# aluo7/ViT-SOM

Measured on AMD Instinct MI355X. Metric: images/sec/node ViT-SOM 40x40 CIFAR-10 bs512 (training step: fwd+bwd+all-reduce+AdamW), higher is better.
Workload: dtype f32 (Linear GEMMs on bf16 MFMA: forward from an exact 3xbf16 operand split, six products; weight / input gradients from a 2xbf16 split, three products, rel. error 4e-6)

## Files before the change

vit_som_amd/csrc/attention.hip:

```cpp
#include "common.h"
#include "attention_layout.h"

#include <atomic>

#include <stdlib.h>

#pragma clang fp contract(off)

namespace vsom {

int gemm_grad_products();

static std::atomic<int> g_attn_fused{1};

#ifdef VSOM_ATTN_STAMPS
__device__ unsigned long long* g_attn_stamps = nullptr;
#define ATTN_STAMP(i)                                                                              \
    do {                                                                                           \
        if (threadIdx.x == 0 && g_attn_stamps) g_attn_stamps[blockIdx.x * 16 + (i)] = __builtin_amdgcn_s_memrealtime(); \
    } while (0)
#define ATTN_STAMP_HWID()                                                                          \
    do {                                                                                           \
        if (threadIdx.x == 0 && g_attn_stamps) {                                                   \
            unsigned hw, xcc;                                                                      \
            asm volatile("s_getreg_b32 %0, hwreg(HW_REG_HW_ID)" : "=s"(hw));                       \
            asm volatile("s_getreg_b32 %0, hwreg(HW_REG_XCC_ID)" : "=s"(xcc));                     \
            g_attn_stamps[blockIdx.x * 16 + 4] = hw;                                                \
            g_attn_stamps[blockIdx.x * 16 + 5] = xcc;                                               \
        }                                                                                          \
    } while (0)
#else
#define ATTN_STAMP(i)
#define ATTN_STAMP_HWID()
#endif


template <int HDP>
struct ACfg {
    static constexpr bool VEC = (HDP % 16 == 0);
    static constexpr int S = HDP + 4;
    static constexpr int NMM = HDP / 4;
    static constexpr int NDT = (HDP + 15) / 16;
    static __device__ __forceinline__ int off(int row, int col) { return row * S + col; }
};

__device__ __forceinline__ f32x4 mfma16(float a, float b, f32x4 c) {
    return __builtin_amdgcn_mfma_f32_16x16x4f32(a, b, c, 0, 0, 0);
}

typedef __attribute__((ext_vector_type(8))) __bf16 abf16x8;
typedef __attribute__((ext_vector_type(2))) __bf16 abf16x2;
struct SplitFrag { abf16x8 hi[2], lo[2]; };
__device__ __forceinline__ void split8(const float (&v)[8], abf16x8& hi, abf16x8& lo) {
    unsigned h[4], l[4];
#pragma unroll
    for (int e = 0; e < 4; ++e) {
        const abf16x2 a = {(__bf16)v[2 * e], (__bf16)v[2 * e + 1]};
        const unsigned u = __builtin_bit_cast(unsigned, a);
        const float r0 = v[2 * e] - __uint_as_float(u << 16), r1 = v[2 * e + 1] - __uint_as_float(u & 0xffff0000u);
        const abf16x2 b = {(__bf16)r0, (__bf16)r1};
        h[e] = u; l[e] = __builtin_bit_cast(unsigned, b);
    }
    typedef unsigned u32x4v __attribute__((ext_vector_type(4)));
    hi = __builtin_bit_cast(abf16x8, (u32x4v){h[0], h[1], h[2], h[3]});
    lo = __builtin_bit_cast(abf16x8, (u32x4v){l[0], l[1], l[2], l[3]});
}
__device__ __forceinline__ void split_frag(const float (&f)[16], SplitFrag& o) {
#pragma unroll
    for (int m = 0; m < 2; ++m) {
        float v[8];
#pragma unroll
        for (int j = 0; j < 8; ++j) v[j] = f[8 * m + j];
        split8(v, o.hi[m], o.lo[m]);
    }
}
__device__ __forceinline__ void accum_x3_pair(f32x4 (&o)[4], const float* Zlds, int rowa, int rowb, int r, int qp, f32x4 pa, f32x4 pb) {
    const float pv[8] = {pa[0], pa[1], pa[2], pa[3], pb[0], pb[1], pb[2], pb[3]};
    abf16x8 bh, bl;
    split8(pv, bh, bl);
#pragma unroll
    for (int dt = 0; dt < 4; ++dt) {
        float zv[8];
#pragma unroll
        for (int j = 0; j < 4; ++j) {
            zv[j] = Zlds[ACfg<64>::off(rowa + 4 * qp + j, 16 * dt + r)];
            zv[4 + j] = Zlds[ACfg<64>::off(rowb + 4 * qp + j, 16 * dt + r)];
        }
        abf16x8 ah, al;
        split8(zv, ah, al);
        o[dt] = __builtin_amdgcn_mfma_f32_16x16x32_bf16(al, bh, o[dt], 0, 0, 0);
        o[dt] = __builtin_amdgcn_mfma_f32_16x16x32_bf16(ah, bl, o[dt], 0, 0, 0);
        o[dt] = __builtin_amdgcn_mfma_f32_16x16x32_bf16(ah, bh, o[dt], 0, 0, 0);
    }
}
__device__ __forceinline__ f32x4 score_x3(const SplitFrag& a, const SplitFrag& b) {
    f32x4 acc = {0.f, 0.f, 0.f, 0.f};
#pragma unroll
    for (int m = 0; m < 2; ++m) {
        acc = __builtin_amdgcn_mfma_f32_16x16x32_bf16(a.lo[m], b.hi[m], acc, 0, 0, 0);
        acc = __builtin_amdgcn_mfma_f32_16x16x32_bf16(a.hi[m], b.lo[m], acc, 0, 0, 0);
        acc = __builtin_amdgcn_mfma_f32_16x16x32_bf16(a.hi[m], b.hi[m], acc, 0, 0, 0);
    }
    return acc;
}
struct SplitFrag3 { abf16x8 hi[2], lo[2], rest[2]; };
__device__ __forceinline__ void split_frag3(const float (&f)[16], SplitFrag3& o) {
#pragma unroll
    for (int m = 0; m < 2; ++m) {
        float v[8], w[8];
#pragma unroll
        for (int j = 0; j < 8; ++j) v[j] = f[8 * m + j];
        split8(v, o.hi[m], o.lo[m]);
        const abf16x8 h = o.hi[m], l = o.lo[m];
        abf16x8 t;
#pragma unroll
        for (int j = 0; j < 8; ++j) { w[j] = (v[j] - (float)h[j]) - (float)l[j]; t[j] = (__bf16)w[j]; }
        o.rest[m] = t;
    }
}
__device__ __forceinline__ f32x4 score_x6(const SplitFrag3& a, const SplitFrag3& b) {
    f32x4 acc = {0.f, 0.f, 0.f, 0.f};
#pragma unroll
    for (int m = 0; m < 2; ++m) {
        acc = __builtin_amdgcn_mfma_f32_16x16x32_bf16(a.rest[m], b.hi[m], acc, 0, 0, 0);
        acc = __builtin_amdgcn_mfma_f32_16x16x32_bf16(a.hi[m], b.rest[m], acc, 0, 0, 0);
        acc = __builtin_amdgcn_mfma_f32_16x16x32_bf16(a.lo[m], b.lo[m], acc, 0, 0, 0);
        acc = __builtin_amdgcn_mfma_f32_16x16x32_bf16(a.lo[m], b.hi[m], acc, 0, 0, 0);
        acc = __builtin_amdgcn_mfma_f32_16x16x32_bf16(a.hi[m], b.lo[m], acc, 0, 0, 0);
        acc = __builtin_amdgcn_mfma_f32_16x16x32_bf16(a.hi[m], b.hi[m], acc, 0, 0, 0);
    }
    return acc;
}
typedef SplitFrag3 ScoreFrag;
__device__ __forceinline__ void split_score(const float (&f)[16], ScoreFrag& o) { split_frag3(f, o); }
__device__ __forceinline__ f32x4 score_qk(const ScoreFrag& a, const ScoreFrag& b) { return score_x6(a, b); }
typedef unsigned u32x2 __attribute__((ext_vector_type(2)));
__device__ __forceinline__ void swap16(float v, float& a, float& b) {
    const u32x2 t = __builtin_amdgcn_permlane16_swap(__float_as_uint(v), __float_as_uint(v), false, false);
    a = __uint_as_float(t[0]); b = __uint_as_float(t[1]);
}
__device__ __forceinline__ void swap32(float v, float& a, float& b) {
    const u32x2 t = __builtin_amdgcn_permlane32_swap(__float_as_uint(v), __float_as_uint(v), false, false);
    a = __uint_as_float(t[0]); b = __uint_as_float(t[1]);
}
__device__ __forceinline__ float group_sum(float v) {
    float a, b;
    swap16(v, a, b); v = a + b;
    swap32(v, a, b); return a + b;
}
__device__ __forceinline__ float group_max(float v) {
    float a, b;
    swap16(v, a, b); v = fmaxf(a, b);
    swap32(v, a, b); return fmaxf(a, b);
}
template <int CTRL>
__device__ __forceinline__ float dpp_row(float v) {
    return __int_as_float(__builtin_amdgcn_update_dpp(0, __float_as_int(v), CTRL, 0xf, 0xf, false));
}
__device__ __forceinline__ float tile_sum(float v) {
    v += dpp_row<0x128>(v); v += dpp_row<0x124>(v); v += dpp_row<0x122>(v); v += dpp_row<0x121>(v);
    return v;
}
__device__ __forceinline__ float tile_max(float v) {
    v = fmaxf(v, dpp_row<0x128>(v)); v = fmaxf(v, dpp_row<0x124>(v));
    v = fmaxf(v, dpp_row<0x122>(v)); v = fmaxf(v, dpp_row<0x121>(v));
    return v;
}
__device__ __forceinline__ float wave_sum64(float v) { return group_sum(tile_sum(v)); }
template <bool EXTRA>
__device__ __forceinline__ int tok(int t, int r) { return (EXTRA ? 1 : 0) + 16 * t + r; }

template <int HDP>
__device__ __forceinline__ void stage_rows(float* lds, const float* __restrict__ src, long rs, int N, int nrows,
                                           int hd) {
    constexpr int S = ACfg<HDP>::S;
// ... 91 lines not shown
#pragma unroll
            for (int s = 0; s < 4; ++s) f[4 * g + s] = v[s];
        }
    } else {
#pragma unroll
        for (int mm = 0; mm < ACfg<HDP>::NMM; ++mm) {
            const int d = 4 * mm + qp;
            f[mm] = (ok && d < hd) ? rowptr[d] : 0.f;
        }
    }
}

template <int HDP>
__device__ __forceinline__ void load_frag_lds(float (&f)[ACfg<HDP>::NMM], const float* Y, int row, int qp) {
    if constexpr (ACfg<HDP>::VEC) {
#pragma unroll
        for (int g = 0; g < HDP / 16; ++g) {
            const f32x4 v = *reinterpret_cast<const f32x4*>(Y + ACfg<HDP>::off(row, 16 * g + 4 * qp));
#pragma unroll
            for (int s = 0; s < 4; ++s) f[4 * g + s] = v[s];
        }
    } else {
        load_frag<HDP>(f, Y + row * ACfg<HDP>::S, qp, true, HDP);
    }
}

template <int HDP>
__device__ __forceinline__ f32x4 score_tile(const float* Ylds, int row0, int r, int qp,
                                            const float (&bf)[ACfg<HDP>::NMM]) {
    float af[ACfg<HDP>::NMM];
    load_frag_lds<HDP>(af, Ylds, row0 + r, qp);
    f32x4 acc = {0.f, 0.f, 0.f, 0.f};
#pragma unroll
    for (int mm = 0; mm < ACfg<HDP>::NMM; ++mm) acc = mfma16(af[mm], bf[mm], acc);
    return acc;
}
template <int HDP>
__device__ __forceinline__ void score_tile2(const float* Y0, int row0, const float (&b0)[ACfg<HDP>::NMM], const float* Y1,
                                            int row1, const float (&b1)[ACfg<HDP>::NMM], int r, int qp, f32x4& acc0,
                                            f32x4& acc1) {
    float a0[ACfg<HDP>::NMM], a1[ACfg<HDP>::NMM];
    load_frag_lds<HDP>(a0, Y0, row0 + r, qp);
    load_frag_lds<HDP>(a1, Y1, row1 + r, qp);
    acc0 = f32x4{0.f, 0.f, 0.f, 0.f};
    acc1 = f32x4{0.f, 0.f, 0.f, 0.f};
#pragma unroll
    for (int mm = 0; mm < ACfg<HDP>::NMM; ++mm) {
        acc0 = mfma16(a0[mm], b0[mm], acc0);
        acc1 = mfma16(a1[mm], b1[mm], acc1);
    }
}

template <int HDP>
__device__ __forceinline__ void accum_tile(f32x4 (&o)[ACfg<HDP>::NDT], const float* Zlds, int row0, int r, int qp,
                                           f32x4 p) {
#pragma unroll
    for (int s = 0; s < 4; ++s) {
#pragma unroll
        for (int dt = 0; dt < ACfg<HDP>::NDT; ++dt) {
            float a = 0.f;
            if (ACfg<HDP>::VEC || 16 * dt + r < HDP) a = Zlds[ACfg<HDP>::off(row0 + 4 * qp + s, 16 * dt + r)];
            o[dt] = mfma16(a, p[s], o[dt]);
        }
    }
}
template <int HDP>
__device__ __forceinline__ void accum_tile2(f32x4 (&o0)[ACfg<HDP>::NDT], const float* Z0, f32x4 p0,
                                            f32x4 (&o1)[ACfg<HDP>::NDT], const float* Z1, f32x4 p1, int row0, int r,
                                            int qp) {
#pragma unroll
    for (int s = 0; s < 4; ++s) {
#pragma unroll
        for (int dt = 0; dt < ACfg<HDP>::NDT; ++dt) {
            float a0 = 0.f, a1 = 0.f;
            if (ACfg<HDP>::VEC || 16 * dt + r < HDP) {
                a0 = Z0[ACfg<HDP>::off(row0 + 4 * qp + s, 16 * dt + r)];
                a1 = Z1[ACfg<HDP>::off(row0 + 4 * qp + s, 16 * dt + r)];
            }
            o0[dt] = mfma16(a0, p0[s], o0[dt]);
            o1[dt] = mfma16(a1, p1[s], o1[dt]);
        }
    }
}

template <int HDP>
__device__ __forceinline__ void store_rows(const f32x4 (&o)[ACfg<HDP>::NDT], float* dst, int qp, bool ok, int hd) {
    if (!ok) return;
#pragma unroll
    for (int dt = 0; dt < ACfg<HDP>::NDT; ++dt) {
        const int d0 = 16 * dt + 4 * qp;
        if constexpr (ACfg<HDP>::VEC) {
            *reinterpret_cast<f32x4*>(dst + d0) = o[dt];
        } else {
#pragma unroll
            for (int e = 0; e < 4; ++e)
                if (d0 + e < hd) dst[d0 + e] = o[dt][e];
        }
    }
}

template <int HDP>
__device__ __forceinline__ float frag_dot_row(const float (&f)[ACfg<HDP>::NMM], const float* rowptr, int qp) {
    float y[ACfg<HDP>::NMM];
    load_frag<HDP>(y, rowptr, qp, true, HDP);
    float s = 0.f;
#pragma unroll
    for (int mm = 0; mm < ACfg<HDP>::NMM; ++mm) s = fmaf(f[mm], y[mm], s);
    return group_sum(s);
}
template <int HDP>
__device__ __forceinline__ void axpy_row(f32x4 (&o)[ACfg<HDP>::NDT], float w, const float* rowptr, int qp) {
#pragma unroll
    for (int dt = 0; dt < ACfg<HDP>::NDT; ++dt) {
        const int d0 = 16 * dt + 4 * qp;
        f32x4 v = {0.f, 0.f, 0.f, 0.f};
        if constexpr (ACfg<HDP>::VEC) {
            v = *reinterpret_cast<const f32x4*>(rowptr + d0);
        } else {
#pragma unroll
            for (int e = 0; e < 4; ++e)
                if (d0 + e < HDP) v[e] = rowptr[d0 + e];
        }
        o[dt] += w * v;
    }
}
template <int HDP>
__device__ __forceinline__ float tile_rows_dot(const float* x, const float* Y, int row0, int r, int qp) {
    float xf[ACfg<HDP>::NMM], y[ACfg<HDP>::NMM];
    load_frag<HDP>(xf, x, qp, true, HDP);
    load_frag_lds<HDP>(y, Y, row0 + r, qp);
    float s = 0.f;
#pragma unroll
    for (int mm = 0; mm < ACfg<HDP>::NMM; ++mm) s = fmaf(xf[mm], y[mm], s);
    return group_sum(s);
}
template <int HDP>
__device__ __forceinline__ float tile_wsum(float w, const float* Z, int row0, int lane) {
    float acc = 0.f;
#pragma unroll 4
    for (int j = 0; j < 16; ++j) {
        const float wj = __int_as_float(__builtin_amdgcn_readlane(__float_as_int(w), j));
        if (HDP >= 64 || lane < HDP) acc = fmaf(wj, Z[ACfg<HDP>::off(row0 + j, lane)], acc);
    }
    return acc;
}
template <int HDP>
__device__ __forceinline__ float vec_dot(const float* x, const float* y, int lane) {
    return wave_sum64((HDP >= 64 || lane < HDP) ? x[lane] * y[lane] : 0.f);
}
template <int HDP>
__device__ __forceinline__ float tok0_dq_partial(const float* q0f, const float* do0f, const float* Ks, const float* Vs, int row0, float l0, float D0,
                                                 float scale, int lane, int r, int qp) {
    const float sc = tile_rows_dot<HDP>(q0f, Ks, row0, r, qp);
    const float dp = tile_rows_dot<HDP>(do0f, Vs, row0, r, qp);
    const float w = __expf(sc * scale - l0) * (dp - D0) * scale;
    return tile_wsum<HDP>(w, Ks, row0, lane);
}
template <int HDP>
__device__ __forceinline__ void tok0_dq_combine(const float* q0, const float* do0, const float* k0, const float* v0,
                                                const float* PA, int pa_stride, int nwaves, float l0, float D0,
                                                float scale, float* dst, int hd, int lane) {
    const float s00 = vec_dot<HDP>(q0, k0, lane);
    const float dp00 = vec_dot<HDP>(do0, v0, lane);
    const float w00 = __expf(s00 * scale - l0) * (dp00 - D0) * scale;
    if (HDP >= 64 || lane < HDP) {
        float g = w00 * k0[lane];
        for (int w = 0; w < nwaves; ++w) g += PA[w * pa_stride + lane];
        if (lane < hd) dst[lane] = g;
    }
}
template <int HDP>
__device__ __forceinline__ void tok0_dkv_partial(const float* k0f, const float* v0f, const float* Qs, const float* Ds, const float* Ls, const float* Es,
                                                 int row0, float scale, int lane, int r, int qp, float& gk, float& gv) {
    const float sc = tile_rows_dot<HDP>(k0f, Qs, row0, r, qp);
    const float dp = tile_rows_dot<HDP>(v0f, Ds, row0, r, qp);
    const float p = __expf(sc * scale - Ls[row0 + r]);
    const float ds = p * (dp - Es[row0 + r]) * scale;
    gv += tile_wsum<HDP>(p, Ds, row0, lane);
    gk += tile_wsum<HDP>(ds, Qs, row0, lane);
}
template <int HDP>
__device__ __forceinline__ void tok0_dkv_combine(const float* q0, const float* do0, const float* k0, const float* v0,
                                                 const float* PA, int pa_stride, int nwaves, float l0, float D0,
                                                 float scale, float* dk_dst, float* dv_dst, int hd, int lane) {
    const float s00 = vec_dot<HDP>(q0, k0, lane);
    const float dp00 = vec_dot<HDP>(do0, v0, lane);
    const float p00 = __expf(s00 * scale - l0);
    const float ds00 = p00 * (dp00 - D0) * scale;
    if (HDP >= 64 || lane < HDP) {
        float gk = ds00 * q0[lane], gv = p00 * do0[lane];
        for (int w = 0; w < nwaves; ++w) {
            gk += PA[w * pa_stride + lane];
            gv += PA[w * pa_stride + HDP + lane];
        }
        if (lane < hd) {
            dk_dst[lane] = gk;
            dv_dst[lane] = gv;
        }
    }
}

template <int HDP>
__device__ __forceinline__ float rows_dot(const float (&a)[ACfg<HDP>::NMM], const float (&b)[ACfg<HDP>::NMM]) {
    float D = 0.f;
#pragma unroll
    for (int mm = 0; mm < ACfg<HDP>::NMM; ++mm) D = fmaf(a[mm], b[mm], D);
    return group_sum(D);
}
template <int HDP>
__device__ __forceinline__ void dq_key0(f32x4 (&dq)[ACfg<HDP>::NDT], const float (&qf)[ACfg<HDP>::NMM],
                                        const float (&dof)[ACfg<HDP>::NMM], const float* Ks, const float* Vs, float lq, float D,
                                        float scale, int qp) {
    const float s0 = frag_dot_row<HDP>(qf, Ks, qp) * scale;
    const float dp0 = frag_dot_row<HDP>(dof, Vs, qp);
    const float p0 = __expf(s0 - lq);
    axpy_row<HDP>(dq, p0 * (dp0 - D) * scale, Ks, qp);
}
template <int HDP, bool EXTRA>
__device__ __forceinline__ void dq_scores(f32x4& p, f32x4& ds, const float (&qf)[ACfg<HDP>::NMM],
                                          const float (&dof)[ACfg<HDP>::NMM], const float* Ks, const float* Vs, int t, int N,
                                          bool qok, float lq, float D, float scale, int r, int qp) {
    f32x4 s, dp;
    score_tile2<HDP>(Ks, tok<EXTRA>(t, 0), qf, Vs, tok<EXTRA>(t, 0), dof, r, qp, s, dp);
#pragma unroll
    for (int e = 0; e < 4; ++e) {
        const int key = tok<EXTRA>(t, 4 * qp + e);
        p[e] = (EXTRA || (key < N && qok)) ? __expf(s[e] * scale - lq) : 0.f;
        ds[e] = p[e] * (dp[e] - D) * scale;
    }
}
template <int HDP, bool EXTRA>
__device__ __forceinline__ void dq_tile(f32x4 (&dq)[ACfg<HDP>::NDT], const float (&qf)[ACfg<HDP>::NMM],
                                        const float (&dof)[ACfg<HDP>::NMM], const float* Ks, const float* Vs, int ntile, int N,
                                        bool qok, float lq, float D, float scale, int r, int qp) {
#pragma unroll
    for (int dt = 0; dt < ACfg<HDP>::NDT; ++dt) dq[dt] = f32x4{0.f, 0.f, 0.f, 0.f};
    if (EXTRA) dq_key0<HDP>(dq, qf, dof, Ks, Vs, lq, D, scale, qp);
    for (int t = 0; t < ntile; ++t) {
        f32x4 p, ds;
        dq_scores<HDP, EXTRA>(p, ds, qf, dof, Ks, Vs, t, N, qok, lq, D, scale, r, qp);
        accum_tile<HDP>(dq, Ks, tok<EXTRA>(t, 0), r, qp, ds);
    }
}
template <int HDP, bool EXTRA>
__device__ __forceinline__ void dkv_tile(f32x4 (&dk)[ACfg<HDP>::NDT], f32x4 (&dv)[ACfg<HDP>::NDT],
                                         const float (&kf)[ACfg<HDP>::NMM], const float (&vf)[ACfg<HDP>::NMM], const float* Qs,
                                         const float* Ds, const float* Ls, const float* Es, int ntile, int N, bool kok,
                                         float scale, int r, int qp) {
#pragma unroll
    for (int dt = 0; dt < ACfg<HDP>::NDT; ++dt) { dk[dt] = f32x4{0.f, 0.f, 0.f, 0.f}; dv[dt] = f32x4{0.f, 0.f, 0.f, 0.f}; }
    if (EXTRA) {
        const float s0 = frag_dot_row<HDP>(kf, Qs, qp) * scale;
        const float dp0 = frag_dot_row<HDP>(vf, Ds, qp);
        const float p0 = __expf(s0 - Ls[0]);
        axpy_row<HDP>(dv, p0, Ds, qp);
        axpy_row<HDP>(dk, p0 * (dp0 - Es[0]) * scale, Qs, qp);
    }
    for (int t = 0; t < ntile; ++t) {
        f32x4 s, dp;
        score_tile2<HDP>(Qs, tok<EXTRA>(t, 0), kf, Ds, tok<EXTRA>(t, 0), vf, r, qp, s, dp);
        f32x4 p, ds;
#pragma unroll
// ... 319 lines not shown
    {
        const int q0 = tok<EXTRA>(wave, r);
        load_frag<HDP>(qf, base + (long)q0 * E3, qp, q0 < N, hd);
        load_frag<HDP>(dof, dout + obase + (long)q0 * E, qp, q0 < N, hd);
        load_frag<HDP>(of, out + obase + (long)q0 * E, qp, q0 < N, hd);
    }
    float o0 = 0.f;
    if (EXTRA && lane < hd) o0 = out[obase + lane];
    float l_r = 0.f;
    if ((int)threadIdx.x < N) l_r = lse[srow0 + threadIdx.x];
    stage_rows_quad<HDP>(Ks, base + E, E3, Vs, base + 2 * E, E3, Qs, base, E3, Ds, dout + obase, E, N, nrows);
    for (int i = threadIdx.x; i < nrp; i += blockDim.x) {
        Ls[i] = (i == (int)threadIdx.x) ? l_r : ((i < N) ? lse[srow0 + i] : 0.f);
        Es[i] = 0.f;
    }
    __syncthreads();
    ATTN_STAMP(1);
#ifdef VSOM_ATTN_REPEAT
    for (int rep_ = 0; rep_ < VSOM_ATTN_REPEAT; ++rep_) {
    __syncthreads();
#endif

    float D0 = 0.f, l0 = 0.f, gq0 = 0.f;
    if (EXTRA) {
        D0 = wave_sum64((HDP >= 64 || lane < HDP) ? Ds[lane] * o0 : 0.f);
        l0 = Ls[0];
        if (wave == 0 && lane == 0) { delta[srow0] = D0; Es[0] = D0; }
    }
    for (int qt = wave; qt < ntile; qt += nwaves) {
        const int query = tok<EXTRA>(qt, r);
        const bool qok = query < N;
        if (qt != wave) {
            load_frag<HDP>(qf, base + (long)query * E3, qp, qok, hd);
            load_frag<HDP>(dof, dout + obase + (long)query * E, qp, qok, hd);
            load_frag<HDP>(of, out + obase + (long)query * E, qp, qok, hd);
        }
        const float D = rows_dot<HDP>(dof, of);
        if (qp == 0 && qok) { delta[srow0 + query] = D; Es[query] = D; }
        const float lq = qok ? Ls[query] : 0.f;
        f32x4 dq[NDT];
        dq_tile<HDP, EXTRA>(dq, qf, dof, Ks, Vs, ntile, N, qok, lq, D, scale, r, qp);
        store_rows<HDP>(dq, dqkv + ((long)b * N + query) * E3 + h * hd, qp, qok, hd);
        if (EXTRA) gq0 += tok0_dq_partial<HDP>(Qs, Ds, Ks, Vs, tok<EXTRA>(qt, 0), l0, D0, scale, lane, r, qp);
    }
    if (EXTRA && (HDP >= 64 || lane < HDP)) PA[wave * lay.paw + lane] = gq0;
    __syncthreads();
    ATTN_STAMP(2);

    float gk0 = 0.f, gv0 = 0.f;
    if (EXTRA && wave == 0)
        tok0_dq_combine<HDP>(Qs, Ds, Ks, Vs, PA, lay.paw, nwaves, l0, D0, scale, dqkv + (long)b * N * E3 + h * hd, hd, lane);
    for (int kt = wave; kt < ntile; kt += nwaves) {
        const int key = tok<EXTRA>(kt, r);
        const bool kok = key < N;
        float kf[NMM], vf[NMM];
        load_frag_lds<HDP>(kf, Ks, key, qp);
        load_frag_lds<HDP>(vf, Vs, key, qp);
        f32x4 dk[NDT], dv[NDT];
        dkv_tile<HDP, EXTRA>(dk, dv, kf, vf, Qs, Ds, Ls, Es, ntile, N, kok, scale, r, qp);
        float* drow = dqkv + ((long)b * N + key) * E3 + h * hd;
        store_rows<HDP>(dk, drow + E, qp, kok, hd);
        store_rows<HDP>(dv, drow + 2 * E, qp, kok, hd);
        if (EXTRA) tok0_dkv_partial<HDP>(Ks, Vs, Qs, Ds, Ls, Es, tok<EXTRA>(kt, 0), scale, lane, r, qp, gk0, gv0);
    }
    if (EXTRA) {
        if (HDP >= 64 || lane < HDP) {
            PA[wave * lay.paw + HDP + lane] = gk0;
            PA[wave * lay.paw + 2 * HDP + lane] = gv0;
        }
        __syncthreads();
        if (wave == 0) {
            float* drow = dqkv + (long)b * N * E3 + h * hd;
            tok0_dkv_combine<HDP>(Qs, Ds, Ks, Vs, PA + HDP, lay.paw, nwaves, Ls[0], Es[0], scale, drow + E, drow + 2 * E, hd,
                                  lane);
        }
    }
#ifdef VSOM_ATTN_REPEAT
    }
#endif
    ATTN_STAMP(3);
}

template <int HDP, bool EXTRA, bool BF16X3 = false>
__global__ __launch_bounds__(256) void attn_bwd_shared_kernel(const float* __restrict__ qkv, const float* __restrict__ out,
                                                              const float* __restrict__ dout, const float* __restrict__ lse,
                                                              float* __restrict__ dqkv, float* __restrict__ delta, int N,
                                                              int H, int hd, float scale) {
    extern __shared__ __attribute__((aligned(16))) float smem[];
    constexpr int NDT = ACfg<HDP>::NDT;
    constexpr int NMM = ACfg<HDP>::NMM;
    const int b = blockIdx.x / H, h = blockIdx.x % H;
    const int E = H * hd, E3 = 3 * E;
    const int lane = threadIdx.x & 63, wave = threadIdx.x >> 6, nwaves = blockDim.x >> 6;
    const int r = lane & 15, qp = lane >> 4;
    constexpr int S = ACfg<HDP>::S;
    const int ntile = EXTRA ? (N - 1) >> 4 : (N + 15) >> 4;
    const int nrows = EXTRA ? N : ntile << 4;
    const int nrp = (nrows + 3) & ~3;
    const int PS = 16 * ntile + 4;
    float* Ks = smem;
    float* Vs = Ks + nrows * S;
    float* Qs = Vs + nrows * S;
    float* Ds = Qs + nrows * S;
    float* Ls = Ds + nrows * S;
    float* Es = Ls + nrp;
    float* PA = Es + nrp;
    float* X2 = PA + (blockDim.x >> 6) * 3 * HDP;
    float* X3 = X2 + HDP;
    float* Pm = Ks;
    float* Dm = Vs;
    const float* base = qkv + (long)b * N * E3 + h * hd;
    const long obase = (long)b * N * E + h * hd;
    const long srow0 = ((long)b * H + h) * N;
    float qf[NMM], dof[NMM], of[NMM];
    ATTN_STAMP(0);
    ATTN_STAMP_HWID();
    const int own = tok<EXTRA>(wave, r);
    const bool ook = own < N;
    load_frag<HDP>(qf, base + (long)own * E3, qp, ook, hd);
    load_frag<HDP>(dof, dout + obase + (long)own * E, qp, ook, hd);
    if constexpr (!(BF16X3 && HDP == 64)) load_frag<HDP>(of, out + obase + (long)own * E, qp, ook, hd);
    float o0 = 0.f;
    if (EXTRA && lane < hd) o0 = out[obase + lane];
    float l_r = 0.f;
    if ((int)threadIdx.x < N) l_r = lse[srow0 + threadIdx.x];
    stage_rows_quad<HDP>(Ks, base + E, E3, Vs, base + 2 * E, E3, Qs, base, E3, Ds, dout + obase, E, N, nrows);
    for (int i = threadIdx.x; i < nrp; i += blockDim.x) {
        Ls[i] = (i == (int)threadIdx.x) ? l_r : ((i < N) ? lse[srow0 + i] : 0.f);
        Es[i] = 0.f;
    }
    __syncthreads();
    ATTN_STAMP(1);

    float D0 = 0.f, l0 = 0.f, gq0 = 0.f;
    if (EXTRA) {
        D0 = wave_sum64((HDP >= 64 || lane < HDP) ? Ds[lane] * o0 : 0.f);
        l0 = Ls[0];
        if (wave == 0 && lane == 0) { delta[srow0] = D0; Es[0] = D0; }
    }
    f32x4 pT[4], dsT[4];
    ScoreFrag qs;
    SplitFrag dos;
    if constexpr (BF16X3 && HDP == 64) { split_score(qf, qs); split_frag(dof, dos); }
    {
        const int query = own;
        const bool qok = ook;
        const float lq = qok ? Ls[query] : 0.f;
        f32x4 dq[NDT];
#pragma unroll
        for (int dt = 0; dt < NDT; ++dt) dq[dt] = f32x4{0.f, 0.f, 0.f, 0.f};
        if constexpr (BF16X3 && HDP == 64) {
            float s0 = 0.f, dp0 = 0.f, p0 = 0.f, dsum = 0.f, mx = -INFINITY, z = 0.f;
            if (EXTRA) {
                s0 = frag_dot_row<HDP>(qf, Ks, qp) * scale;
                dp0 = frag_dot_row<HDP>(dof, Vs, qp);
                mx = s0;
            }
            f32x4 dpT[4];
#pragma unroll
            for (int t = 0; t < 4; ++t) {
                if (t < ntile) {
                    float kf[16], vf[16];
                    load_frag_lds<HDP>(kf, Ks, tok<EXTRA>(t, 0) + r, qp);
                    load_frag_lds<HDP>(vf, Vs, tok<EXTRA>(t, 0) + r, qp);
                    ScoreFrag ka;
                    SplitFrag va;
                    split_score(kf, ka);
                    split_frag(vf, va);
                    const f32x4 sc = score_qk(ka, qs);
                    dpT[t] = score_x3(va, dos);
#pragma unroll
                    for (int e = 0; e < 4; ++e) {
                        const int key = tok<EXTRA>(t, 4 * qp + e);
                        pT[t][e] = (EXTRA || key < N) ? sc[e] * scale : -INFINITY;
                        mx = fmaxf(mx, pT[t][e]);
                    }
                }
            }
            mx = group_max(mx);
#pragma unroll
            for (int t = 0; t < 4; ++t) {
                if (t < ntile) {
#pragma unroll
                    for (int e = 0; e < 4; ++e) {
                        const float p = qok ? __expf(pT[t][e] - mx) : 0.f;
                        pT[t][e] = p;
                        z += p;
                        dsum = fmaf(p, dpT[t][e], dsum);
                    }
                }
            }
            z = group_sum(z);
            dsum = group_sum(dsum);
            if (EXTRA) {
                p0 = qok ? __expf(s0 - mx) : 0.f;
                z += p0;
                dsum = fmaf(p0, dp0, dsum);
            }
            const float inv = qok ? 1.0f / z : 0.f;
            p0 *= inv;
#pragma unroll
            for (int t = 0; t < 4; ++t)
                if (t < ntile) pT[t] *= inv;
            const float D = dsum * inv;
            if (qp == 0 && qok) { delta[srow0 + query] = D; Es[query] = D; }
            if (EXTRA) axpy_row<HDP>(dq, p0 * (dp0 - D) * scale, Ks, qp);
#pragma unroll
            for (int t = 0; t < 4; ++t) {
                if (t < ntile) {
#pragma unroll
                    for (int e = 0; e < 4; ++e) dsT[t][e] = pT[t][e] * (dpT[t][e] - D) * scale;
                    if (t & 1) accum_x3_pair(dq, Ks, tok<EXTRA>(t - 1, 0), tok<EXTRA>(t, 0), r, qp, dsT[t - 1], dsT[t]);
                    else if (t + 1 >= ntile) accum_tile<HDP>(dq, Ks, tok<EXTRA>(t, 0), r, qp, dsT[t]);
                }
            }
        } else {
            const float D = rows_dot<HDP>(dof, of);
            if (qp == 0 && qok) { delta[srow0 + query] = D; Es[query] = D; }
            if (EXTRA) dq_key0<HDP>(dq, qf, dof, Ks, Vs, lq, D, scale, qp);
#pragma unroll
            for (int t = 0; t < 4; ++t) {
                if (t < ntile) {
                    dq_scores<HDP, EXTRA>(pT[t], dsT[t], qf, dof, Ks, Vs, t, N, qok, lq, D, scale, r, qp);
                    accum_tile<HDP>(dq, Ks, tok<EXTRA>(t, 0), r, qp, dsT[t]);
                }
            }
        }
        store_rows<HDP>(dq, dqkv + ((long)b * N + query) * E3 + h * hd, qp, qok, hd);
        if (EXTRA) gq0 += tok0_dq_partial<HDP>(Qs, Ds, Ks, Vs, tok<EXTRA>(wave, 0), l0, D0, scale, lane, r, qp);
    }
    if (EXTRA && (HDP >= 64 || lane < HDP)) PA[wave * 3 * HDP + lane] = gq0;
    __syncthreads();
    ATTN_STAMP(2);

    float gk0 = 0.f, gv0 = 0.f, p0k = 0.f, w0k = 0.f;
    if (EXTRA) {
        if (wave == 0)
            tok0_dq_combine<HDP>(Qs, Ds, Ks, Vs, PA, 3 * HDP, nwaves, l0, D0, scale, dqkv + (long)b * N * E3 + h * hd, hd, lane);
        float kf[NMM], vf[NMM];
        load_frag_lds<HDP>(kf, Ks, own, qp);
        load_frag_lds<HDP>(vf, Vs, own, qp);
        const float s0 = frag_dot_row<HDP>(kf, Qs, qp) * scale;
        const float dp0 = frag_dot_row<HDP>(vf, Ds, qp);
        p0k = __expf(s0 - Ls[0]);
        w0k = p0k * (dp0 - Es[0]) * scale;
        if (wave == nwaves - 1 && (HDP >= 64 || lane < HDP)) { X2[lane] = Ks[lane]; X3[lane] = Vs[lane]; }
    }
    __syncthreads();
#pragma unroll
    for (int t = 0; t < 4; ++t)
        if (t < ntile) {
            *reinterpret_cast<f32x4*>(Pm + (16 * wave + r) * PS + 16 * t + 4 * qp) = pT[t];
            *reinterpret_cast<f32x4*>(Dm + (16 * wave + r) * PS + 16 * t + 4 * qp) = dsT[t];
        }
    __syncthreads();

    {
        const int key = own;
        const bool kok = ook;
        f32x4 dk[NDT], dv[NDT];
#pragma unroll
        for (int dt = 0; dt < NDT; ++dt) { dk[dt] = f32x4{0.f, 0.f, 0.f, 0.f}; dv[dt] = f32x4{0.f, 0.f, 0.f, 0.f}; }
        if (EXTRA) {
            axpy_row<HDP>(dv, p0k, Ds, qp);
            axpy_row<HDP>(dk, w0k, Qs, qp);
        }
        for (int t = 0; t < ntile; ++t) {
            f32x4 p, ds;
#pragma unroll
            for (int e = 0; e < 4; ++e) {
                p[e] = Pm[(16 * t + 4 * qp + e) * PS + 16 * wave + r];
                ds[e] = Dm[(16 * t + 4 * qp + e) * PS + 16 * wave + r];
            }
            if constexpr (BF16X3 && HDP == 64) {
                if (t + 1 < ntile) {
                    f32x4 p1, ds1;
#pragma unroll
                    for (int e = 0; e < 4; ++e) {
                        p1[e] = Pm[(16 * (t + 1) + 4 * qp + e) * PS + 16 * wave + r];
                        ds1[e] = Dm[(16 * (t + 1) + 4 * qp + e) * PS + 16 * wave + r];
                    }
                    accum_x3_pair(dv, Ds, tok<EXTRA>(t, 0), tok<EXTRA>(t + 1, 0), r, qp, p, p1);
                    accum_x3_pair(dk, Qs, tok<EXTRA>(t, 0), tok<EXTRA>(t + 1, 0), r, qp, ds, ds1);
                    ++t;
                    continue;
                }
            }
            accum_tile2<HDP>(dv, Ds, p, dk, Qs, ds, tok<EXTRA>(t, 0), r, qp);
        }
        float* drow = dqkv + ((long)b * N + key) * E3 + h * hd;
        store_rows<HDP>(dk, drow + E, qp, kok, hd);
        store_rows<HDP>(dv, drow + 2 * E, qp, kok, hd);
        if (EXTRA) tok0_dkv_partial<HDP>(X2, X3, Qs, Ds, Ls, Es, tok<EXTRA>(wave, 0), scale, lane, r, qp, gk0, gv0);
    }
    if (EXTRA) {
        if (HDP >= 64 || lane < HDP) {
            PA[wave * 3 * HDP + HDP + lane] = gk0;
            PA[wave * 3 * HDP + 2 * HDP + lane] = gv0;
        }
        __syncthreads();
        if (wave == 0) {
            float* drow = dqkv + (long)b * N * E3 + h * hd;
            tok0_dkv_combine<HDP>(Qs, Ds, X2, X3, PA + HDP, 3 * HDP, nwaves, Ls[0], Es[0], scale, drow + E, drow + 2 * E, hd, lane);
        }
    }
    ATTN_STAMP(3);
}

static bool use_extra(int N) { return N >= 17 && (N % 16) == 1; }
static int attn_tiles(int N) { return use_extra(N) ? (N - 1) / 16 : cdiv(N, 16); }
static int attn_waves(int N) {
    const int ntile = attn_tiles(N);
    if (ntile >= 8) return 8;
    return ntile > 4 ? 4 : ntile;
}
static int attn_hdp(int hd) {
    if (hd == 16 || hd == 32 || hd == 64) return hd;
    if (hd >= 1 && hd <= 4) return 4;
    if (hd <= 8) return 8;
    return 0;
}
static size_t attn_lds_bytes(int N, int hdp, AttnLds kind) {
    return AttnLayout<size_t>(0, N, hdp, use_extra(N), attn_waves(N), kind).end * sizeof(float);
}
static size_t attn_shared_lds_bytes(int N, int hdp) { return attn_lds_bytes(N, hdp, ATTN_LDS_FUSED) + 2 * hdp * sizeof(float); }

template <int HDP, bool EXTRA>
static int launch_fwd_t(const float* qkv, float* out, float* lse, int B, int N, int H, int hd, hipStream_t st) {
    const size_t lds = attn_lds_bytes(N, HDP, ATTN_LDS_FWD);
    VSOM_LAUNCH((attn_fwd_kernel<HDP, EXTRA>), dim3(B * H), dim3(64 * attn_waves(N)), lds, st, qkv, out, lse, N, H, hd,
                       1.0f / sqrtf((float)hd));
    return launch_status("attn_fwd_kernel");
}
enum AttnBwd : int { ATTN_BWD_TWO_LAUNCH = 0, ATTN_BWD_FUSED = 1, ATTN_BWD_SHARED = 2, ATTN_BWD_SHARED_BF16X3 = 3 };
static AttnBwd attn_bwd_plan(int N, int hdp, int hook, int grad_products) {
    const bool vec = hdp % 16 == 0;
    const AttnLayout<size_t> fused(0, N, hdp, use_extra(N), attn_waves(N), ATTN_LDS_FUSED);
    const int nt = fused.ntile, nrows = fused.nrows;
    if (vec && (hook == 1 || hook == 3) && nt <= 4 && attn_waves(N) == nt && 16 * nt * (16 * nt + 4) <= nrows * (hdp + 4) &&
        attn_shared_lds_bytes(N, hdp) <= 80 * 1024)
        return (hdp == 64 && grad_products == 3 && hook == 1) ? ATTN_BWD_SHARED_BF16X3 : ATTN_BWD_SHARED;
    if (vec && hook != 0 && fused.end * sizeof(float) <= 80 * 1024) return ATTN_BWD_FUSED;
    return ATTN_BWD_TWO_LAUNCH;
}

int attn_bwd_threads(int N) { return 64 * attn_waves(N); }
int attn_bwd_plan_now(int N, int hd) {
    const int hdp = attn_hdp(hd);
    return hdp ? (int)attn_bwd_plan(N, hdp, g_attn_fused.load(std::memory_order_relaxed), gemm_grad_products()) : -1;
}

template <int HDP, bool EXTRA>
static int launch_bwd_t(const float* qkv, const float* out, const float* dout, const float* lse, float* dqkv,
                        float* delta, int B, int N, int H, int hd, hipStream_t st) {
    const float scale = 1.0f / sqrtf((float)hd);
    const dim3 grid(B * H), block(64 * attn_waves(N));
    const AttnBwd plan = attn_bwd_plan(N, HDP, g_attn_fused.load(std::memory_order_relaxed), gemm_grad_products());
    switch (plan) {
        case ATTN_BWD_SHARED_BF16X3:
            if constexpr (HDP == 64) {
                VSOM_LAUNCH((attn_bwd_shared_kernel<HDP, EXTRA, true>), grid, block, attn_shared_lds_bytes(N, HDP), st,
                            qkv, out, dout, lse, dqkv, delta, N, H, hd, scale);
                return launch_status("attn_bwd_shared_kernel");
            }
            break;
        case ATTN_BWD_SHARED:
            if constexpr (ACfg<HDP>::VEC) {
                VSOM_LAUNCH((attn_bwd_shared_kernel<HDP, EXTRA>), grid, block, attn_shared_lds_bytes(N, HDP), st, qkv,
                            out, dout, lse, dqkv, delta, N, H, hd, scale);
                return launch_status("attn_bwd_shared_kernel");
            }
            break;
        case ATTN_BWD_FUSED:
            if constexpr (ACfg<HDP>::VEC) {
                VSOM_LAUNCH((attn_bwd_fused_kernel<HDP, EXTRA>), grid, block, attn_lds_bytes(N, HDP, ATTN_LDS_FUSED), st, qkv,
                            out, dout, lse, dqkv, delta, N, H, hd, scale);
                return launch_status("attn_bwd_fused_kernel");
            }
            break;
        case ATTN_BWD_TWO_LAUNCH: {
            VSOM_LAUNCH((attn_bwd_dq_kernel<HDP, EXTRA>), grid, block, attn_lds_bytes(N, HDP, ATTN_LDS_DQ), st, qkv, out,
                        dout, lse, dqkv, delta, N, H, hd, scale);
            const int rc = launch_status("attn_bwd_dq_kernel");
            if (rc) return rc;
            VSOM_LAUNCH((attn_bwd_dkv_kernel<HDP, EXTRA>), grid, block, attn_lds_bytes(N, HDP, ATTN_LDS_DKV), st, qkv,
                        dout, lse, delta, dqkv, N, H, hd, scale);
            return launch_status("attn_bwd_dkv_kernel");
        }
    }
    set_error("attention_bwd: plan %d has no kernel at head dim %d", (int)plan, HDP);
    return VSOM_EUNSUPPORTED;
}
template <int HDP>
static int launch_fwd(const float* qkv, float* out, float* lse, int B, int N, int H, int hd, hipStream_t st) {
    return use_extra(N) ? launch_fwd_t<HDP, true>(qkv, out, lse, B, N, H, hd, st)
                        : launch_fwd_t<HDP, false>(qkv, out, lse, B, N, H, hd, st);
}
template <int HDP>
static int launch_bwd(const float* qkv, const float* out, const float* dout, const float* lse, float* dqkv,
                      float* delta, int B, int N, int H, int hd, hipStream_t st) {
    return use_extra(N) ? launch_bwd_t<HDP, true>(qkv, out, dout, lse, dqkv, delta, B, N, H, hd, st)
                        : launch_bwd_t<HDP, false>(qkv, out, dout, lse, dqkv, delta, B, N, H, hd, st);
}


__global__ __launch_bounds__(256) void attn_probs_kernel(const float* __restrict__ qkv, float* __restrict__ probs, int N, int H,
                                                         int hd, float scale) {
    const int bh = blockIdx.x, b = bh / H, h = bh % H;
    const int E3 = 3 * H * hd;
    const int lane = threadIdx.x & 63, wave = threadIdx.x >> 6;
    const float* q0 = qkv + (long)b * N * E3 + h * hd;
    const float* k0 = q0 + H * hd;
    for (int i = blockIdx.y * 4 + wave; i < N; i += gridDim.y * 4) {
        const float* q = q0 + (long)i * E3;
        float* p = probs + ((long)bh * N + i) * N;
        float m = -INFINITY;
        for (int j = lane; j < N; j += 64) {
            const float* k = k0 + (long)j * E3;
            float s = 0.f;
            for (int d = 0; d < hd; ++d) s = fmaf(q[d], k[d], s);
            s *= scale;
            p[j] = s;
            m = fmaxf(m, s);
        }
        m = wave_max(m);
        float z = 0.f;
        for (int j = lane; j < N; j += 64) {
            const float e = __expf(p[j] - m);
            p[j] = e;
            z += e;
        }
        const float inv = 1.0f / wave_sum(z);
        for (int j = lane; j < N; j += 64) p[j] *= inv;
    }
}

static int attn_check(const char* who, int B, int N, int H, int hd, int* hdp) {
    VSOM_REQUIRE(B > 0 && N > 0 && H > 0 && hd > 0, VSOM_EINVAL, "%s: bad shape B=%d N=%d H=%d hd=%d", who, B, N, H, hd);
    *hdp = attn_hdp(hd);
    VSOM_REQUIRE(*hdp != 0, VSOM_EUNSUPPORTED, "%s: head dim %d not supported (1..8, 16, 32, 64)", who, hd);
    const size_t lds = attn_lds_bytes(N, *hdp, ATTN_LDS_DKV);
    VSOM_REQUIRE(lds <= 160 * 1024, VSOM_EUNSUPPORTED, "%s: N=%d hd=%d needs %zu B of LDS (> 160 KiB)", who, N, hd, lds);
    return VSOM_OK;
}
// ... 54 lines not shown
```

Before: 58700.

## Stream Q and dO from global in bf16x3 attention backward to shrink LDS

In the bf16x3 shared attention backward kernel (hd=64), Q and dO are no longer staged into LDS. The dK/dV accumulation and the token-0 partials now read them directly from global memory through buffer loads, with the loads software-pipelined against the split-bf16 MFMAs. The kernel also gets a waves-per-EU hint of 3, and the launch uses a smaller LDS footprint, with the goal of raising occupancy. The cost is repeated global/L2 reads and higher register pressure, which could spill or lower memory efficiency.

```diff
diff --git a/vit_som_amd/csrc/attention.hip b/vit_som_amd/csrc/attention.hip
--- a/vit_som_amd/csrc/attention.hip
+++ b/vit_som_amd/csrc/attention.hip
@@ -13,6 +13,9 @@
 
 static std::atomic<int> g_attn_fused{1};
 
+#ifndef VSOM_ATTN_KV_PAD
+#define VSOM_ATTN_KV_PAD 0
+#endif
 #ifdef VSOM_ATTN_STAMPS
 __device__ unsigned long long* g_attn_stamps = nullptr;
 #define ATTN_STAMP(i)                                                                              \
@@ -74,6 +77,13 @@
         split8(v, o.hi[m], o.lo[m]);
     }
 }
+__device__ __forceinline__ f32x4 accum_x3_dt(f32x4 o, const float (&zv)[8], abf16x8 bh, abf16x8 bl) {
+    abf16x8 ah, al;
+    split8(zv, ah, al);
+    o = __builtin_amdgcn_mfma_f32_16x16x32_bf16(al, bh, o, 0, 0, 0);
+    o = __builtin_amdgcn_mfma_f32_16x16x32_bf16(ah, bl, o, 0, 0, 0);
+    return __builtin_amdgcn_mfma_f32_16x16x32_bf16(ah, bh, o, 0, 0, 0);
+}
 __device__ __forceinline__ void accum_x3_pair(f32x4 (&o)[4], const float* Zlds, int rowa, int rowb, int r, int qp, f32x4 pa, f32x4 pb) {
     const float pv[8] = {pa[0], pa[1], pa[2], pa[3], pb[0], pb[1], pb[2], pb[3]};
     abf16x8 bh, bl;
@@ -86,11 +96,33 @@
             zv[j] = Zlds[ACfg<64>::off(rowa + 4 * qp + j, 16 * dt + r)];
             zv[4 + j] = Zlds[ACfg<64>::off(rowb + 4 * qp + j, 16 * dt + r)];
         }
-        abf16x8 ah, al;
-        split8(zv, ah, al);
-        o[dt] = __builtin_amdgcn_mfma_f32_16x16x32_bf16(al, bh, o[dt], 0, 0, 0);
-        o[dt] = __builtin_amdgcn_mfma_f32_16x16x32_bf16(ah, bl, o[dt], 0, 0, 0);
-        o[dt] = __builtin_amdgcn_mfma_f32_16x16x32_bf16(ah, bh, o[dt], 0, 0, 0);
+        o[dt] = accum_x3_dt(o[dt], zv, bh, bl);
+    }
+}
+__device__ __forceinline__ float bload1(__amdgpu_buffer_rsrc_t rs, unsigned off) {
+    return __builtin_bit_cast(float, __builtin_amdgcn_raw_buffer_load_b32(rs, (int)off, 0, 0));
+}
+__device__ __forceinline__ void global_pair(float (&z)[32], __amdgpu_buffer_rsrc_t rs, unsigned rsb, int rowa, int rowb, int r, int qp) {
+#pragma unroll
+    for (int j = 0; j < 4; ++j) {
+        const unsigned oa = (unsigned)(rowa + 4 * qp + j) * rsb + 4u * r, ob = (unsigned)(rowb + 4 * qp + j) * rsb + 4u * r;
+#pragma unroll
+        for (int dt = 0; dt < 4; ++dt) {
+            z[8 * dt + j] = bload1(rs, oa + 64u * dt);
+            z[8 * dt + 4 + j] = bload1(rs, ob + 64u * dt);
+        }
+    }
+}
+__device__ __forceinline__ void accum_x3_vals(f32x4 (&o)[4], const float (&z)[32], f32x4 pa, f32x4 pb) {
+    const float pv[8] = {pa[0], pa[1], pa[2], pa[3], pb[0], pb[1], pb[2], pb[3]};
+    abf16x8 bh, bl;
+    split8(pv, bh, bl);
+#pragma unroll
+    for (int dt = 0; dt < 4; ++dt) {
+        float zv[8];
+#pragma unroll
+        for (int j = 0; j < 8; ++j) zv[j] = z[8 * dt + j];
+        o[dt] = accum_x3_dt(o[dt], zv, bh, bl);
     }
 }
 __device__ __forceinline__ f32x4 score_x3(const SplitFrag& a, const SplitFrag& b) {
@@ -348,6 +380,28 @@
         }
     }
 }
+__device__ __forceinline__ void accum_tile2_global(f32x4 (&o0)[4], __amdgpu_buffer_rsrc_t rs0, unsigned rsb0, f32x4 p0,
+                                                   f32x4 (&o1)[4], __amdgpu_buffer_rsrc_t rs1, unsigned rsb1, f32x4 p1,
+                                                   int row0, int r, int qp) {
+    float a0[16], a1[16];
+#pragma unroll
+    for (int s = 0; s < 4; ++s) {
+        const unsigned q0 = (unsigned)(row0 + 4 * qp + s) * rsb0 + 4u * r, q1 = (unsigned)(row0 + 4 * qp + s) * rsb1 + 4u * r;
+#pragma unroll
+        for (int dt = 0; dt < 4; ++dt) {
+            a0[4 * s + dt] = bload1(rs0, q0 + 64u * dt);
+            a1[4 * s + dt] = bload1(rs1, q1 + 64u * dt);
+        }
+    }
+#pragma unroll
+    for (int s = 0; s < 4; ++s) {
+#pragma unroll
+        for (int dt = 0; dt < 4; ++dt) {
+            o0[dt] = mfma16(a0[4 * s + dt], p0[s], o0[dt]);
+            o1[dt] = mfma16(a1[4 * s + dt], p1[s], o1[dt]);
+        }
+    }
+}
 
 template <int HDP>
 __device__ __forceinline__ void store_rows(const f32x4 (&o)[ACfg<HDP>::NDT], float* dst, int qp, bool ok, int hd) {
@@ -444,6 +498,36 @@
     const float ds = p * (dp - Es[row0 + r]) * scale;
     gv += tile_wsum<HDP>(p, Ds, row0, lane);
     gk += tile_wsum<HDP>(ds, Qs, row0, lane);
+}
+template <int HDP>
+__device__ __forceinline__ float tile_rows_dot_global(const float* x, const float* Yrow, int qp) {
+    float xf[ACfg<HDP>::NMM], y[ACfg<HDP>::NMM];
+    load_frag<HDP>(xf, x, qp, true, HDP);
+    load_frag<HDP>(y, Yrow, qp, true, HDP);
+    float s = 0.f;
+#pragma unroll
+    for (int mm = 0; mm < ACfg<HDP>::NMM; ++mm) s = fmaf(xf[mm], y[mm], s);
+    return group_sum(s);
+}
+template <int HDP>
+__device__ __forceinline__ float tile_wsum_global(float w, const float* Z, long rs, int lane) {
+    float z[16], acc = 0.f;
+#pragma unroll
+    for (int j = 0; j < 16; ++j) z[j] = Z[j * rs + lane];
+#pragma unroll
+    for (int j = 0; j < 16; ++j) acc = fmaf(__int_as_float(__builtin_amdgcn_readlane(__float_as_int(w), j)), z[j], acc);
+    return acc;
+}
+template <int HDP>
+__device__ __forceinline__ void tok0_dkv_partial_global(const float* k0f, const float* v0f, const float* Qg, long rsq, const float* Dg, long rsd,
+                                                        const float* Ls, const float* Es, int row0, float scale, int lane, int r, int qp,
+                                                        float& gk, float& gv) {
+    const float sc = tile_rows_dot_global<HDP>(k0f, Qg + r * rsq, qp);
+    const float dp = tile_rows_dot_global<HDP>(v0f, Dg + r * rsd, qp);
+    const float p = __expf(sc * scale - Ls[row0 + r]);
+    const float ds = p * (dp - Es[row0 + r]) * scale;
+    gv += tile_wsum_global<HDP>(p, Dg, rsd, lane);
+    gk += tile_wsum_global<HDP>(ds, Qg, rsq, lane);
 }
 template <int HDP>
 __device__ __forceinline__ void tok0_dkv_combine(const float* q0, const float* do0, const float* k0, const float* v0,
@@ -929,7 +1013,7 @@
 }
 
 template <int HDP, bool EXTRA, bool BF16X3 = false>
-__global__ __launch_bounds__(256) void attn_bwd_shared_kernel(const float* __restrict__ qkv, const float* __restrict__ out,
+__global__ __launch_bounds__(256) __attribute__((amdgpu_waves_per_eu(BF16X3 ? 3 : 1))) void attn_bwd_shared_kernel(const float* __restrict__ qkv, const float* __restrict__ out,
                                                               const float* __restrict__ dout, const float* __restrict__ lse,
                                                               float* __restrict__ dqkv, float* __restrict__ delta, int N,
                                                               int H, int hd, float scale) {
@@ -945,15 +1029,18 @@
     const int nrows = EXTRA ? N : ntile << 4;
     const int nrp = (nrows + 3) & ~3;
     const int PS = 16 * ntile + 4;
+    constexpr bool KV = BF16X3 && HDP == 64;
     float* Ks = smem;
     float* Vs = Ks + nrows * S;
     float* Qs = Vs + nrows * S;
     float* Ds = Qs + nrows * S;
     float* Ls = Ds + nrows * S;
+    if constexpr (KV) Ls = Vs + nrows * S;
     float* Es = Ls + nrp;
     float* PA = Es + nrp;
     float* X2 = PA + (blockDim.x >> 6) * 3 * HDP;
     float* X3 = X2 + HDP;
+    if constexpr (KV) { Qs = X3 + HDP; Ds = Qs + HDP; }
     float* Pm = Ks;
     float* Dm = Vs;
     const float* base = qkv + (long)b * N * E3 + h * hd;
@@ -971,7 +1058,14 @@
     if (EXTRA && lane < hd) o0 = out[obase + lane];
     float l_r = 0.f;
     if ((int)threadIdx.x < N) l_r = lse[srow0 + threadIdx.x];
-    stage_rows_quad<HDP>(Ks, base + E, E3, Vs, base + 2 * E, E3, Qs, base, E3, Ds, dout + obase, E, N, nrows);
+    if constexpr (KV) {
+        float q0 = 0.f, do0 = 0.f;
+        if (EXTRA && threadIdx.x < HDP) { q0 = base[threadIdx.x]; do0 = dout[obase + threadIdx.x]; }
+        stage_rows_pair<HDP>(Ks, base + E, E3, Vs, base + 2 * E, E3, N, nrows, hd);
+        if (EXTRA && threadIdx.x < HDP) { Qs[threadIdx.x] = q0; Ds[threadIdx.x] = do0; }
+    } else {
+        stage_rows_quad<HDP>(Ks, base + E, E3, Vs, base + 2 * E, E3, Qs, base, E3, Ds, dout + obase, E, N, nrows);
+    }
     for (int i = threadIdx.x; i < nrp; i += blockDim.x) {
         Ls[i] = (i == (int)threadIdx.x) ? l_r : ((i < N) ? lse[srow0 + i] : 0.f);
         Es[i] = 0.f;
@@ -1112,33 +1206,53 @@
             axpy_row<HDP>(dv, p0k, Ds, qp);
             axpy_row<HDP>(dk, w0k, Qs, qp);
         }
-        for (int t = 0; t < ntile; ++t) {
-            f32x4 p, ds;
-#pragma unroll
-            for (int e = 0; e < 4; ++e) {
-                p[e] = Pm[(16 * t + 4 * qp + e) * PS + 16 * wave + r];
-                ds[e] = Dm[(16 * t + 4 * qp + e) * PS + 16 * wave + r];
-            }
-            if constexpr (BF16X3 && HDP == 64) {
-                if (t + 1 < ntile) {
-                    f32x4 p1, ds1;
-#pragma unroll
-                    for (int e = 0; e < 4; ++e) {
-                        p1[e] = Pm[(16 * (t + 1) + 4 * qp + e) * PS + 16 * wave + r];
-                        ds1[e] = Dm[(16 * (t + 1) + 4 * qp + e) * PS + 16 * wave + r];
-                    }
-                    accum_x3_pair(dv, Ds, tok<EXTRA>(t, 0), tok<EXTRA>(t + 1, 0), r, qp, p, p1);
-                    accum_x3_pair(dk, Qs, tok<EXTRA>(t, 0), tok<EXTRA>(t + 1, 0), r, qp, ds, ds1);
-                    ++t;
-                    continue;
+        auto pcol = [&](const float* M, int t) {
+            f32x4 v;
+#pragma unroll
+            for (int e = 0; e < 4; ++e) v[e] = M[(16 * t + 4 * qp + e) * PS + 16 * wave + r];
+            return v;
+        };
+        if constexpr (KV) {
+            const __amdgpu_buffer_rsrc_t rq = __builtin_amdgcn_make_buffer_rsrc(const_cast<float*>(base), 0, ((N - 1) * E3 + HDP) * 4, 0x00020000);
+            const __amdgpu_buffer_rsrc_t rd = __builtin_amdgcn_make_buffer_rsrc(const_cast<float*>(dout + obase), 0, ((N - 1) * E + HDP) * 4, 0x00020000);
+            const unsigned sq = E3 * 4, sd = E * 4;
+            float zd[32], zq[32];
+            if (ntile >= 2) {
+                global_pair(zd, rd, sd, tok<EXTRA>(0, 0), tok<EXTRA>(1, 0), r, qp);
+                global_pair(zq, rq, sq, tok<EXTRA>(0, 0), tok<EXTRA>(1, 0), r, qp);
+                accum_x3_vals(dv, zd, pcol(Pm, 0), pcol(Pm, 1));
+                if (ntile >= 4) global_pair(zd, rd, sd, tok<EXTRA>(2, 0), tok<EXTRA>(3, 0), r, qp);
+                accum_x3_vals(dk, zq, pcol(Dm, 0), pcol(Dm, 1));
+                if (ntile >= 4) {
+                    global_pair(zq, rq, sq, tok<EXTRA>(2, 0), tok<EXTRA>(3, 0), r, qp);
+                    accum_x3_vals(dv, zd, pcol(Pm, 2), pcol(Pm, 3));
+                    accum_x3_vals(dk, zq, pcol(Dm, 2), pcol(Dm, 3));
                 }
             }
-            accum_tile2<HDP>(dv, Ds, p, dk, Qs, ds, tok<EXTRA>(t, 0), r, qp);
+            if (ntile & 1)
+                accum_tile2_global(dv, rd, sd, pcol(Pm, ntile - 1), dk, rq, sq, pcol(Dm, ntile - 1), tok<EXTRA>(ntile - 1, 0), r, qp);
+        } else {
+            for (int t = 0; t < ntile; ++t) {
+                f32x4 p, ds;
+#pragma unroll
+                for (int e = 0; e < 4; ++e) {
+                    p[e] = Pm[(16 * t + 4 * qp + e) * PS + 16 * wave + r];
+                    ds[e] = Dm[(16 * t + 4 * qp + e) * PS + 16 * wave + r];
+                }
+                accum_tile2<HDP>(dv, Ds, p, dk, Qs, ds, tok<EXTRA>(t, 0), r, qp);
+            }
         }
         float* drow = dqkv + ((long)b * N + key) * E3 + h * hd;
         store_rows<HDP>(dk, drow + E, qp, kok, hd);
         store_rows<HDP>(dv, drow + 2 * E, qp, kok, hd);
-        if (EXTRA) tok0_dkv_partial<HDP>(X2, X3, Qs, Ds, Ls, Es, tok<EXTRA>(wave, 0), scale, lane, r, qp, gk0, gv0);
+        if (EXTRA) {
+            const int row0 = tok<EXTRA>(wave, 0);
+            if constexpr (KV)
+                tok0_dkv_partial_global<HDP>(X2, X3, base + (long)row0 * E3, E3, dout + obase + (long)row0 * E, E, Ls, Es, row0, scale, lane,
+                                             r, qp, gk0, gv0);
+            else
+                tok0_dkv_partial<HDP>(X2, X3, Qs, Ds, Ls, Es, row0, scale, lane, r, qp, gk0, gv0);
+        }
     }
     if (EXTRA) {
         if (HDP >= 64 || lane < HDP) {
@@ -1171,6 +1285,10 @@
     return AttnLayout<size_t>(0, N, hdp, use_extra(N), attn_waves(N), kind).end * sizeof(float);
 }
 static size_t attn_shared_lds_bytes(int N, int hdp) { return attn_lds_bytes(N, hdp, ATTN_LDS_FUSED) + 2 * hdp * sizeof(float); }
+static size_t attn_shared_kv_lds_bytes(int N, int hdp) {
+    const AttnLayout<size_t> f(0, N, hdp, use_extra(N), attn_waves(N), ATTN_LDS_FUSED);
+    return (f.end - (f.Y3 - f.Y1) + 4 * hdp) * sizeof(float) + VSOM_ATTN_KV_PAD;
+}
 
 template <int HDP, bool EXTRA>
 static int launch_fwd_t(const float* qkv, float* out, float* lse, int B, int N, int H, int hd, hipStream_t st) {
@@ -1206,7 +1324,7 @@
     switch (plan) {
         case ATTN_BWD_SHARED_BF16X3:
             if constexpr (HDP == 64) {
-                VSOM_LAUNCH((attn_bwd_shared_kernel<HDP, EXTRA, true>), grid, block, attn_shared_lds_bytes(N, HDP), st,
+                VSOM_LAUNCH((attn_bwd_shared_kernel<HDP, EXTRA, true>), grid, block, attn_shared_kv_lds_bytes(N, HDP), st,
                             qkv, out, dout, lse, dqkv, delta, N, H, hd, scale);
                 return launch_status("attn_bwd_shared_kernel");
             }
```

After: 59060 (median of 4 runs). Within noise of the previous version (+0.6%).
